# 115dkk/Impulcifer-pip313

Measured on AMD Instinct MI355X. Metric: impulse responses/sec (sweep deconv+FIR), 7.1×2-ear @48kHz, 1/2/4/8 GPU, higher is better.
Workload: dtype f32

## Files before the change

### impulcifer-pip313_amd/csrc/conv_kernels.hip.h

```cpp
#pragma once
#include "fft_regs.hip.h"

namespace imp {

constexpr int kN2 = 4096;
constexpr int kLogN2 = 12;
constexpr int kRowPad = 272;
#ifndef IMP_AB_PREFETCH
#define IMP_AB_PREFETCH 8
#endif
constexpr int kAbPrefetch = IMP_AB_PREFETCH;

struct Twiddles {
  const cf* __restrict__ full;
  const cf* __restrict__ hi;
  const cf* __restrict__ t1;
  const cf* __restrict__ t2;
  const cf* __restrict__ t4;
};

__device__ __forceinline__ void xcd_work_item(int nchan, int& tile, int& chan) {
  const int xcd = blockIdx.x & 7;
  const int slot = blockIdx.x >> 3;
  const int tl = slot / nchan;
// ... 795 lines not shown
#pragma unroll
  for (int q = 1; q < 16; ++q) u[q] = bload_cf(r_t2, vl8, q * 16 * 8);
  fft16<+1>(v);
#pragma unroll
  for (int q = 1; q < 16; ++q) v[q] = cmulc(v[q], u[q]);
  wave_lds_fence();
#pragma unroll
  for (int t2 = 0; t2 < 16; ++t2) buf[hi4 * kRowPad + t2 * 17 + lo4] = v[t2];
  wave_lds_fence();
#pragma unroll
  for (int q = 0; q < 16; ++q) u[q] = buf[hi4 * kRowPad + lo4 * 17 + q];
#pragma unroll
  for (int j2 = 0; j2 < 16; ++j2) v[j2] = bload_cf(r_t4, vo8, j2 * 256 * 8);
  fft16<+1>(u);
#pragma unroll
  for (int j2 = 0; j2 < 16; ++j2) u[j2] = cmulc(u[j2], v[j2]);
  wave_lds_fence();
#pragma unroll
  for (int j2 = 0; j2 < 16; ++j2) buf[hi4 * kRowPad + 16 * j2 + lo4] = u[j2];
  __syncthreads();
#pragma unroll
  for (int a = 0; a < 16; ++a) v[a] = buf[a * kRowPad + t];
  fft16<+1>(v);
#pragma unroll
  for (int j = 0; j < 16; ++j) bstore_cf<IMP_AUX_ROWS_ST>(v[j], r_row, vo8, j * 256 * 8);
}

struct FirBlockArgs {
  const float4* __restrict__ ab;
  long long ab_chan_stride;
  float* __restrict__ out;
  long long out_stride;
  long long out_start, out_len;
  int kp;
  int valid;
  int blocks;
  int first_block;
  int nchan;
};

template <int N1>
struct FirBlockCfg {
  static_assert(N1 == 2 || N1 == 4, "fir_block_kernel holds two or four rows");
  static constexpr int kThreads = 256 * N1;
  static constexpr int kPoints = N1 * kN2;
  static constexpr size_t kLds = sizeof(cf) * N1 * 16 * kRowPad;
  static constexpr int kAbPrefetch = N1 == 4 ? 4 : ::imp::kAbPrefetch;
};
constexpr int kFirBlockPoints = FirBlockCfg<4>::kPoints;
constexpr size_t kFirBlockLds = FirBlockCfg<4>::kLds;

template <class L, class = void> struct LoadHasDeviceLen { static constexpr bool value = false; };
template <class L> struct LoadHasDeviceLen<L, decltype((void)L::kDeviceLen)> { static constexpr bool value = true; };

template <int N1>
__device__ __forceinline__ cf fir_twiddle(__amdgpu_buffer_rsrc_t r_full, int k1, int n2) {
  return bload_cf(r_full, (unsigned)((k1 * (4 / N1)) * kN2 + n2) * 8u, 0u);
}

template <int N1, class Load>
__global__ __launch_bounds__(FirBlockCfg<N1>::kThreads, 4) void fir_block_kernel(Load ld, FirBlockArgs a, Twiddles tw) {
  using Cfg = FirBlockCfg<N1>;
  constexpr int T = Cfg::kThreads;
  extern __shared__ __attribute__((aligned(16))) char smem_raw[];
  cf* lds = reinterpret_cast<cf*>(smem_raw);
  const int xcd = blockIdx.x & 7, slot = blockIdx.x >> 3;
  const int chan = (slot / a.blocks) * 8 + xcd, blk = a.first_block + slot % a.blocks;
  if (chan >= a.nchan) return;
  long long out_len = a.out_len;
  int filt = chan;
  if constexpr (LoadHasDeviceLen<Load>::value) {
    out_len = ld.out_len(chan);
    filt = ld.filter_of(chan);
    if ((long long)blk * a.valid - a.out_start >= out_len) return;
  }
  const int tid = threadIdx.x;
  const int pairq = N1 == 4 ? __builtin_amdgcn_readfirstlane(tid >> 9) : 0;
  const int half = __builtin_amdgcn_readfirstlane((tid >> 8) & 1);
  const int t = tid & 255;
  const int k1 = pairq + (N1 / 2) * half;
  const int s0 = blk * a.valid - a.kp;
  const __amdgpu_buffer_rsrc_t r_full = make_rsrc(tw.full, 4u * kN2 * 8u);
  const auto row = ld.open(chan);

  constexpr int CPT = kN2 / T;
  constexpr int CH = 8 / N1;
  cf v[16];
#pragma unroll
  for (int h = 0; h < CPT / CH; ++h) {
    cf x[CH][N1], w[CH][N1 - 1];
#pragma unroll
    for (int c = 0; c < CH; ++c) {
      const int n2 = tid + T * (CH * h + c);
#pragma unroll
      for (int n1 = 0; n1 < N1; ++n1) x[c][n1] = row.pair_at(s0 + 2 * (n1 * kN2 + n2));
#pragma unroll
      for (int k = 1; k < N1; ++k) w[c][k - 1] = fir_twiddle<N1>(r_full, k, n2);
    }
#pragma unroll
    for (int c = 0; c < CH; ++c) {
      const int n2 = tid + T * (CH * h + c);
#pragma unroll
      for (int n1 = 0; n1 < N1; ++n1) x[c][n1] = row.finish(x[c][n1], s0 + 2 * (n1 * kN2 + n2));
      if constexpr (N1 == 4) bfly4<-1>(x[c][0], x[c][1], x[c][2], x[c][3]);
      else bfly2<-1>(x[c][0], x[c][1]);
      lds[n2] = x[c][0];
#pragma unroll
      for (int k = 1; k < N1; ++k) lds[k * kN2 + n2] = cmul(x[c][k], w[c][k - 1]);
    }
  }
  __syncthreads();
#pragma unroll
  for (int j = 0; j < 16; ++j) v[j] = lds[k1 * kN2 + t + 256 * j];
  __syncthreads();
  const __amdgpu_buffer_rsrc_t r_ab =
      make_rsrc(a.ab + (long long)filt * a.ab_chan_stride + (long long)k1 * kN2, kN2 * sizeof(float4));
  rows_core<0, Cfg::kAbPrefetch>(v, lds + pairq * (2 * 16 * kRowPad), half, pairq, k1, r_ab, tw, t);

  __syncthreads();
#pragma unroll
  for (int j = 0; j < 16; ++j) lds[k1 * kN2 + t + 256 * j] = v[j];
  __syncthreads();
  const __amdgpu_buffer_rsrc_t r_out = make_rsrc(a.out + (long long)chan * a.out_stride, (unsigned)out_len * 4u);
  const int o0 = blk * a.valid - a.kp - (int)a.out_start;
#pragma unroll
  for (int c = 0; c < CPT; ++c) {
    const int n2 = tid + T * c;
    cf y[N1];
#pragma unroll
    for (int k = 0; k < N1; ++k) y[k] = lds[k * kN2 + n2];
#pragma unroll
    for (int k = 1; k < N1; ++k) y[k] = cmulc(y[k], fir_twiddle<N1>(r_full, k, n2));
    if constexpr (N1 == 4) bfly4<+1>(y[0], y[1], y[2], y[3]);
    else bfly2<+1>(y[0], y[1]);
#pragma unroll
    for (int n1 = 0; n1 < N1; ++n1) {
// ... 17 lines not shown
```

### impulcifer-pip313_amd/csrc/impulse_hip.hip

```cpp
#include <hip/hip_runtime.h>

#include <algorithm>
#include <cmath>
#include <complex>
#include <cstdarg>
#include <cstdio>
#include <cstdlib>
#include <cstring>
#include <map>
#include <mutex>
#include <new>
#include <string>
#include <vector>

#include "internal.h"
#include "conv_kernels.hip.h"
#include "ir_kernels.hip.h"
#include "decay_kernels.hip.h"
#include "slice_kernels.hip.h"
#include "vbass_kernels.hip.h"
#include "micdev_kernels.hip.h"

static thread_local std::string g_last_error;

// ... 1674 lines not shown
  return mic_mismatch_impl<float>(ctx, "imp_mic_mismatch_device", d_x, off, len, peak, group, side, anchor, B, G, win, pre, fs, grid,
                                  M, raw_out, power_out);
}

extern "C" int imp_mic_mismatch(imp_ctx* ctx, const double* x, const int64_t* off, const int64_t* len, const int64_t* peak,
                                const int32_t* group, const int32_t* side, const int32_t* anchor, int64_t B, int64_t G, int64_t win,
                                int64_t pre, double fs, const double* grid, int64_t M, double* raw_out, double* power_out) {
  if (!ctx) return fail(IMP_ERR_INVALID, "imp_mic_mismatch: null ctx");
  IMP_CTX_LOCK(ctx);
  int64_t ext = 0;
  int rc = mic_check("imp_mic_mismatch", x, off, len, peak, group, side, anchor, B, G, win, pre, fs, grid, M, raw_out, &ext);
  if (rc || (rc = ctx_bind(ctx))) return rc;
  double* d_x = nullptr;
  if ((rc = ctx_block_get(ctx, (size_t)std::max<int64_t>(ext, 1) * sizeof(double), (void**)&d_x))) return rc;
  if (ext > 0) {
    hipError_t e = hipMemcpyAsync(d_x, x, (size_t)ext * sizeof(double), hipMemcpyHostToDevice, ctx->stream);
    if (e != hipSuccess) {
      (void)hipStreamSynchronize(ctx->stream);
      (void)ctx_block_put(ctx, d_x);
      return fail(IMP_ERR_HIP, "imp_mic_mismatch: h2d: %s", hipGetErrorString(e));
    }
  }
  rc = mic_mismatch_impl<double>(ctx, "imp_mic_mismatch", d_x, off, len, peak, group, side, anchor, B, G, win, pre, fs, grid, M,
                                 raw_out, power_out);
  (void)hipStreamSynchronize(ctx->stream);
  (void)ctx_block_put(ctx, d_x);
  return rc;
}

struct imp_chain {
  imp_ctx* ctx = nullptr;
  imp_ctx* tail_ctx = nullptr;
  imp_plan* deconv = nullptr;
  imp_plan* fir = nullptr;
  int64_t B = 0, n = 0, head = 0, fade_in = 0, fade_out = 0, pitch_ir = 0;
  double peak_height = 0.12589;
  int lanes = 1;
  int sets = 1;
  int64_t calls = 0;
  int tiles = 0;
  int64_t chunks = 0;
  std::vector<float*> d_ir;
  std::vector<unsigned*> d_tile;
  std::vector<imp::RowPeak*> d_res;
  std::vector<hipEvent_t> k1_done;
  std::vector<hipEvent_t> ir_free;
  std::vector<char> ir_busy;
  int64_t* d_meta = nullptr;
  double* d_win = nullptr;
  float4* d_ab2 = nullptr;
  int64_t ab2_gen = -1;
  int t2_kp = 0, t2_valid = 0;
  int64_t t2_first = 0, t2_blocks = 0;
};

static bool chain_tail2_geometry(int64_t M, int64_t out_start, int64_t out_len, int* kp, int* valid, int64_t* first,
                                 int64_t* blocks) {
  if (M < 1 || M > kChainTail2MaxTaps) return false;
  *kp = (int)((M - 1 + 1) & ~(int64_t)1);
  *valid = (int)(2 * imp::FirBlockCfg<2>::kPoints - *kp);
  *first = out_start / *valid;
  *blocks = (out_start + out_len - 1) / *valid - *first + 1;
  return true;
}

static int chain_tail2_prepare(imp_chain* c, bool* ready) {
  imp_plan* f = c->fir;
  *ready = false;
  if (!c->d_ab2) return IMP_OK;
  if (c->ab2_gen == f->filter_gen) {
    *ready = true;
    return IMP_OK;
  }
  if (!f->d_taps || f->taps_gen != f->filter_gen) return IMP_OK;
  int rc = spectrum_alpha_beta_device(f->ctx, f->d_taps, f->M, f->n_filters, f->M, imp::FirBlockCfg<2>::kPoints, 2, c->d_ab2, true);
  if (rc) return rc;
  c->ab2_gen = f->filter_gen;
  *ready = true;
  return IMP_OK;
}

struct ChainLock {
  std::unique_lock<std::recursive_mutex> a, b;
  ChainLock(imp_ctx* x, imp_ctx* y) {
    if (x == y) {
      a = std::unique_lock<std::recursive_mutex>(x->mu);
    } else {
      imp_ctx* lo = x < y ? x : y;
      imp_ctx* hi = x < y ? y : x;
      a = std::unique_lock<std::recursive_mutex>(lo->mu);
      b = std::unique_lock<std::recursive_mutex>(hi->mu);
    }
  }
};

extern "C" void imp_chain_destroy(imp_chain* c) {
  if (!c) return;
  ChainLock lk(c->ctx, c->tail_ctx);
  (void)hipSetDevice(c->ctx->device);
  (void)plan_sync_lanes(c->deconv);
  (void)hipStreamSynchronize(c->tail_ctx->stream);
  for (auto p : c->d_ir) (void)hipFree(p);
  for (auto p : c->d_tile) (void)hipFree(p);
  for (auto p : c->d_res) (void)hipFree(p);
  for (auto e : c->k1_done) (void)hipEventDestroy(e);
  for (auto e : c->ir_free) (void)hipEventDestroy(e);
// ... 30 lines not shown
    return fail(IMP_ERR_UNSUPPORTED, "imp_chain_create: deconvolution plan of %d rows", deconv->N1);
  int rc = ctx_bind(deconv->ctx);
  if (rc) return rc;
  imp_chain* c = new (std::nothrow) imp_chain();
  if (!c) return fail(IMP_ERR_ALLOC, "out of host memory");
  c->ctx = deconv->ctx;
  c->tail_ctx = fir->ctx;
  c->deconv = deconv;
  c->fir = fir;
  c->B = B;
  c->n = n;
  c->head = head;
  c->fade_in = fade_in;
  c->fade_out = fade_out;
  c->peak_height = peak_height;
  c->lanes = deconv->lanes;
  c->sets = deconv->ctx == fir->ctx ? 1 : c->lanes + 1;
  c->pitch_ir = (deconv->out_len + 63) / 64 * 64;
  std::vector<int64_t> meta((size_t)(2 * B));
  for (int64_t b = 0; b < B; ++b) {
    meta[(size_t)b] = b * c->pitch_ir;
    meta[(size_t)(B + b)] = deconv->out_len;
  }
  c->tiles = plan_col_tiles(deconv);
  c->chunks = deconv->paired ? deconv->N1 / 2 : deconv->N1;
  const size_t chunk_bytes = (size_t)(B * c->chunks) * sizeof(unsigned);
  bool ok = hipMalloc((void**)&c->d_meta, (size_t)(2 * B) * sizeof(int64_t)) == hipSuccess &&
            hipMemcpy(c->d_meta, meta.data(), meta.size() * sizeof(int64_t), hipMemcpyHostToDevice) == hipSuccess &&
            hipMalloc((void**)&c->d_win, (size_t)std::max<int64_t>(fade_in + fade_out, 1) * sizeof(double)) == hipSuccess;
  if (ok && fade_in + fade_out > 0) {
    hipLaunchKernelGGL(imp::fade_table_kernel, dim3((unsigned)((fade_in + fade_out + 255) / 256)), dim3(256), 0, deconv->ctx->stream,
                       c->d_win, (long long)fade_in, (long long)fade_out);
    ok = hipGetLastError() == hipSuccess && hipStreamSynchronize(deconv->ctx->stream) == hipSuccess;
  }
  for (int l = 0; l < c->sets && ok; ++l) {
    float* ir = nullptr;
    unsigned* tile = nullptr;
    imp::RowPeak* res = nullptr;
    hipEvent_t e1 = nullptr, e2 = nullptr;
    ok = hipMalloc((void**)&ir, (size_t)(B * c->pitch_ir) * sizeof(float)) == hipSuccess;
    if (ir) c->d_ir.push_back(ir);
    ok = ok && hipMalloc((void**)&tile, chunk_bytes * (size_t)c->tiles) == hipSuccess;
    if (tile) c->d_tile.push_back(tile);
    ok = ok && hipMalloc((void**)&res, (size_t)B * sizeof(imp::RowPeak)) == hipSuccess;
    if (res) c->d_res.push_back(res);
    ok = ok && hipEventCreateWithFlags(&e1, hipEventDisableTiming) == hipSuccess;
    if (e1) c->k1_done.push_back(e1);
    ok = ok && hipEventCreateWithFlags(&e2, hipEventDisableTiming) == hipSuccess;
    if (e2) c->ir_free.push_back(e2);
  }
  c->ir_busy.assign((size_t)c->sets, 0);
  const char* k5_env = std::getenv("IMPULSE_HIP_CHAIN_K5");
  const bool block4 = k5_env && std::strcmp(k5_env, "block4") == 0;
  if (ok && fir->fused && !block4 &&
      chain_tail2_geometry(fir->M, fir->out_start, fir->out_len, &c->t2_kp, &c->t2_valid, &c->t2_first, &c->t2_blocks)) {
    ok = hipMalloc((void**)&c->d_ab2, (size_t)fir->n_filters * imp::FirBlockCfg<2>::kPoints * sizeof(float4)) == hipSuccess;
    bool ready = false;
    if (ok && (rc = chain_tail2_prepare(c, &ready))) {
      imp_chain_destroy(c);
      return rc;
    }
  }
  if (!ok) {
    (void)hipGetLastError();
    imp_chain_destroy(c);
    return fail(IMP_ERR_ALLOC, "imp_chain_create: device allocation failed");
  }
  *out = c;
  return IMP_OK;
}

extern "C" int imp_chain_execute_device(imp_chain* c, const float* d_x, int64_t chan_stride_in, int64_t elem_stride_in,
                                        float* d_out, int64_t chan_stride_out, long long* d_peaks_out) {
  if (!c || !d_x || !d_out) return fail(IMP_ERR_INVALID, "imp_chain_execute_device: null argument");
  ChainLock lk(c->ctx, c->tail_ctx);
  if (chan_stride_out < c->fir->out_len)
    return fail(IMP_ERR_INVALID, "chan_stride_out %lld < out_len %lld", (long long)chan_stride_out, (long long)c->fir->out_len);
  if (c->deconv->lanes != c->lanes || c->fir->lanes != 1)
    return fail(IMP_ERR_INVALID, "imp_chain_execute_device: a plan's overlap setting changed since the chain was made");
  int rc = ctx_bind(c->ctx);
  if (rc) return rc;
  const int lane = c->lanes > 1 ? (int)(c->deconv->group_counter_lane % c->lanes) : 0;
  const int l = (int)(c->calls++ % c->sets);
  hipStream_t lane_stream = lane ? c->ctx->side_streams[(size_t)(lane - 1)] : c->ctx->stream;
  hipStream_t tail = c->tail_ctx->stream;
  if (c->ir_busy[(size_t)l] && tail != lane_stream) HIP_TRY(hipStreamWaitEvent(lane_stream, c->ir_free[(size_t)l], 0));
  c->deconv->tile_max = c->d_tile[(size_t)l];
  rc = imp_conv_execute_device(c->deconv, d_x, c->B, chan_stride_in, elem_stride_in, c->d_ir[(size_t)l], c->pitch_ir);
  c->deconv->tile_max = nullptr;
  if (rc) return rc;
  if (c->deconv->cur_stream != lane_stream) return fail(IMP_ERR_HIP, "imp_chain_execute_device: lane bookkeeping out of step");
  if (tail != lane_stream) {
    HIP_TRY(hipEventRecord(c->k1_done[(size_t)l], lane_stream));
    HIP_TRY(hipStreamWaitEvent(tail, c->k1_done[(size_t)l], 0));
  }
  hipLaunchKernelGGL(imp::row_first_peak_chunked_kernel, dim3((unsigned)c->B), dim3(imp::kPeakThreads), 0, tail, c->d_ir[(size_t)l],
                     c->d_meta, c->d_meta + c->B, c->deconv->out_start, (const unsigned*)c->d_tile[(size_t)l], c->tiles,
                     (const unsigned*)nullptr, c->chunks, c->d_res[(size_t)l], c->peak_height, d_peaks_out);
  HIP_TRY(hipGetLastError());
  imp::LoadCropAtPeak ld{c->d_ir[(size_t)l], c->pitch_ir, c->deconv->out_len, c->d_res[(size_t)l], c->n, c->head, c->fade_in, c->fade_out,
                         c->d_win};
  bool tail2 = false;
  if ((rc = chain_tail2_prepare(c, &tail2))) return rc;
  if (tail2) {
    imp_plan* f = c->fir;
    f->cur_stream = f->ctx->stream;
    if ((rc = timing_event(f, 0))) return rc;
    if ((rc = launch_fir_block_rows<2>(f, ld, c->B, d_out, chan_stride_out, c->d_ab2, c->t2_kp, c->t2_valid, c->t2_first,
                                       c->t2_blocks)))
      return rc;
    for (int slot = 1; slot <= 3; ++slot)
      if ((rc = timing_event(f, slot))) return rc;
  } else if ((rc = run_group_with(c->fir, ld, c->B, d_out, chan_stride_out, 0, 2))) {
    return rc;
  }
  if (tail != lane_stream) {
    HIP_TRY(hipEventRecord(c->ir_free[(size_t)l], tail));
    c->ir_busy[(size_t)l] = 1;
  }
  return IMP_OK;
}

extern "C" int imp_chain_tail_rows(imp_chain* c, int* rows) {
  if (!c || !rows) return fail(IMP_ERR_INVALID, "imp_chain_tail_rows: null argument");
  ChainLock lk(c->ctx, c->tail_ctx);
  imp_plan* f = c->fir;
  *rows = c->d_ab2 && (c->ab2_gen == f->filter_gen || (f->d_taps && f->taps_gen == f->filter_gen)) ? 2 : 4;
  return IMP_OK;
}

extern "C" int imp_debug_chain_tail_geometry(int64_t M, int64_t L, int64_t* history, int64_t* valid, int64_t* blocks) {
  if (L < 1) return fail(IMP_ERR_INVALID, "L must be >= 1 (got %lld)", (long long)L);
  int kp = 0, v = 0;
  int64_t first = 0, nb = 0;
  if (!chain_tail2_geometry(M, 0, L + M - 1, &kp, &v, &first, &nb))
    return fail(IMP_ERR_UNSUPPORTED, "the chain's 2-row K5 takes 1 to %lld taps (got %lld)", (long long)kChainTail2MaxTaps,
                (long long)M);
  if (history) *history = kp;
  if (valid) *valid = v;
  if (blocks) *blocks = nb;
  return IMP_OK;
}

struct imp_segset {
  imp_ctx* ctx = nullptr;
  int64_t B = 0;
  double* e = nullptr;
  int64_t* off = nullptr;
  int64_t* len = nullptr;
  std::vector<int64_t> h_len;
  void* qbuf = nullptr;
  size_t qcap = 0;
  void* keep_a = nullptr;
  void* keep_b = nullptr;
  std::vector<int64_t> keep_host;
};

extern "C" void imp_segset_destroy(imp_segset* s) {
  if (!s) return;
  IMP_CTX_LOCK(s->ctx);
  (void)hipSetDevice(s->ctx->device);
  (void)hipStreamSynchronize(s->ctx->stream);
  (void)ctx_block_put(s->ctx, s->e);
// ... 775 lines not shown
```

### impulcifer-pip313_amd/csrc/ir_kernels.hip.h

```cpp
#pragma once
#include <hip/hip_runtime.h>
#include <stdint.h>

#include "conv_kernels.hip.h"

namespace imp {

struct RowPeak {
  unsigned int maxabs_bits;
  unsigned int pad;
  unsigned long long first_peak;
  unsigned long long first_max;
};

constexpr int kPeakChunk = 8192;
#ifdef IMP_PEAK_DIAG
#define IMP_PEAK_T(k) do { if (threadIdx.x == 0 && blockIdx.x == 0) peak_ts[k] = clock64(); } while (0)
#else
#define IMP_PEAK_T(k) do { } while (0)
#endif
constexpr int kPeakThreads = 1024;
constexpr int kMaxPlanRows = 256;

__device__ __forceinline__ int64_t peak_chunks(int64_t n, int64_t shift) {
// ... 3 lines not shown
template <int NW>
__device__ __forceinline__ float block_max_f32(float m, float* wm ) {
#pragma unroll
  for (int s = 32; s > 0; s >>= 1) m = fmaxf(m, __shfl_xor(m, s, 64));
  __syncthreads();
  if ((threadIdx.x & 63) == 0) wm[threadIdx.x >> 6] = m;
  __syncthreads();
  float r = wm[0];
#pragma unroll
  for (int k = 1; k < NW; ++k) r = fmaxf(r, wm[k]);
  return r;
}

template <int NW>
__device__ __forceinline__ unsigned long long block_min_u64(unsigned long long v, unsigned long long* wm ) {
#pragma unroll
  for (int s = 32; s > 0; s >>= 1) {
    const unsigned long long o = __shfl_xor(v, s, 64);
    v = o < v ? o : v;
  }
  __syncthreads();
  if ((threadIdx.x & 63) == 0) wm[threadIdx.x >> 6] = v;
  __syncthreads();
  unsigned long long r = wm[0];
#pragma unroll
  for (int k = 1; k < NW; ++k) r = wm[k] < r ? wm[k] : r;
  return r;
}

__global__ __launch_bounds__(256) void row_chunk_max_kernel(const float* __restrict__ x, const int64_t* __restrict__ off,
                                                            const int64_t* __restrict__ len, int64_t shift,
                                                            unsigned* __restrict__ chunk_max, int64_t pitch) {
  const int b = blockIdx.y;
  const int64_t n = len[b], c = blockIdx.x;
  if (c >= peak_chunks(n, shift)) return;
  const int64_t lo = c * kPeakChunk - shift > 0 ? c * kPeakChunk - shift : 0;
  const int64_t hi = (c + 1) * kPeakChunk - shift < n ? (c + 1) * kPeakChunk - shift : n;
  const float* row = x + off[b];
  float m = 0.f;
  int64_t i = lo + threadIdx.x;
  for (; i + 7 * 256 < hi; i += 8 * 256) {
    float v[8];
#pragma unroll
    for (int k = 0; k < 8; ++k) v[k] = row[i + k * 256];
#pragma unroll
    for (int k = 0; k < 8; ++k) m = fmaxf(m, fabsf(v[k]));
  }
  for (; i < hi; i += 256) m = fmaxf(m, fabsf(row[i]));
  __shared__ __attribute__((aligned(16))) float wm[4];
  m = block_max_f32<4>(m, wm);
  if (threadIdx.x == 0) chunk_max[(int64_t)b * pitch + c] = __float_as_uint(m);
}

__global__ __launch_bounds__(kPeakThreads) void row_first_peak_chunked_kernel(
    const float* __restrict__ x, const int64_t* __restrict__ off, const int64_t* __restrict__ len, int64_t shift,
    const unsigned* __restrict__ tile_max, int tiles, const unsigned* __restrict__ chunk_max, int64_t pitch,
    RowPeak* __restrict__ res, double height, long long* __restrict__ peaks_out) {
  const int b = blockIdx.x, tid = threadIdx.x;
#ifdef IMP_PEAK_DIAG
  long long peak_ts[8] = {0, 0, 0, 0, 0, 0, 0, 0};
#endif
  IMP_PEAK_T(0);
  const int64_t n = len[b];
  const float* row = x + off[b];
  const int64_t nch = peak_chunks(n, shift);
  constexpr int NW = kPeakThreads / 64;
  __shared__ __attribute__((aligned(16))) float wmf[NW];
  __shared__ __attribute__((aligned(16))) unsigned long long wmu[NW];
  __shared__ float sx[kPeakChunk + 2];
  constexpr int kLdsChunks = 2048;
  __shared__ unsigned srows[kLdsChunks];
  const unsigned* cm = chunk_max + (int64_t)b * pitch;
  if (tiles > 0) {
    for (int r = tid; r < kMaxPlanRows; r += kPeakThreads) srows[r] = 0u;
    __syncthreads();
    const unsigned* tm = tile_max + (int64_t)b * tiles * pitch;
    const int lane = tid & 63, w = tid >> 6;
    for (int64_t r = lane; r < nch; r += 64) {
      unsigned m = 0u;
#pragma unroll 4
      for (int t = w; t < tiles; t += kPeakThreads / 64) {
        const unsigned v = tm[(int64_t)t * pitch + r];
        m = v > m ? v : m;
      }
      if (m) atomicMax(&srows[r], m);
    }
    __syncthreads();
    cm = srows;
  } else if (nch <= kLdsChunks) {
    for (int64_t c = tid; c < nch; c += kPeakThreads) srows[c] = cm[c];
    __syncthreads();
    cm = srows;
  }
  IMP_PEAK_T(1);
  float mf = 0.f;
  for (int64_t c = tid; c < nch; c += kPeakThreads) mf = fmaxf(mf, __uint_as_float(cm[c]));
  const float maxabs = block_max_f32<NW>(mf, wmf);
  RowPeak out;
  out.maxabs_bits = __float_as_uint(maxabs);
  out.pad = 0u;
  out.first_peak = ~0ull;
  out.first_max = ~0ull;
  if (maxabs >= 1e-20f) {
    __shared__ float s_thr;
    if (tid == 0) {
      const double dmax = (double)maxabs;
      float t = (float)(height * dmax);
      if (!(t >= 0.f)) t = 0.f;
      for (int k = 0; k < 4 && t > 0.f && (double)__uint_as_float(__float_as_uint(t) - 1u) / dmax >= height; ++k)
        t = __uint_as_float(__float_as_uint(t) - 1u);
      for (int k = 0; k < 4 && !((double)t / dmax >= height); ++k) t = __uint_as_float(__float_as_uint(t) + 1u);
      s_thr = t;
    }
    __syncthreads();
    const float thr = s_thr;
    IMP_PEAK_T(2);
    unsigned long long c_q = ~0ull;
    for (int64_t c = tid; c < nch; c += kPeakThreads)
      if (__uint_as_float(cm[c]) >= thr && (unsigned long long)c < c_q) c_q = (unsigned long long)c;
    c_q = block_min_u64<NW>(c_q, wmu);
    constexpr int U = (kPeakChunk + kPeakThreads - 1) / kPeakThreads;
    int64_t lo = 0, hi = 0;
    auto stage = [&](int64_t c) {
      lo = c * kPeakChunk - shift > 0 ? c * kPeakChunk - shift : 0;
      hi = (c + 1) * kPeakChunk - shift < n ? (c + 1) * kPeakChunk - shift : n;
      const int64_t cnt = hi - lo + 2;
      float t[U + 1];
#pragma unroll
      for (int u = 0; u <= U; ++u) {
        const int64_t k = tid + (int64_t)u * kPeakThreads, i = lo - 1 + k;
        t[u] = (k < cnt && i >= 0 && i < n) ? row[i] : 0.f;
      }
      __syncthreads();
#pragma unroll
      for (int u = 0; u <= U; ++u) {
        const int64_t k = tid + (int64_t)u * kPeakThreads;
        if (k < cnt) sx[k] = t[u];
      }
      __syncthreads();
    };
    IMP_PEAK_T(3);
    for (int64_t c = c_q == ~0ull ? nch : (int64_t)c_q; c < nch; ++c) {
      if (!(__uint_as_float(cm[c]) >= thr)) continue;
      stage(c);
      IMP_PEAK_T(4);
      float xs[U];
#pragma unroll
      for (int u = 0; u < U; ++u) {
        const int64_t i = lo + tid + (int64_t)u * kPeakThreads;
        xs[u] = i < hi ? sx[i - lo + 1] : 0.f;
      }
      unsigned long long best = ~0ull;
#pragma unroll
      for (int u = 0; u < U; ++u) {
        const int64_t i = lo + tid + (int64_t)u * kPeakThreads;
        const float xi = xs[u];
        if (best != ~0ull || !(fabsf(xi) >= thr) || i >= hi || i == 0 || i >= n - 1) continue;
        const float xm = sx[i - lo];
        const bool up = xm < xi, dn = xm > xi;
        if (!up && !dn) continue;
        if (!((up ? xi : -xi) >= thr)) continue;
        int64_t j = i;
        while (j + 1 < n && (j + 1 <= hi ? sx[j + 1 - lo + 1] : row[j + 1]) == xi) ++j;
        if (j + 1 >= n) continue;
        const float xn = j + 1 <= hi ? sx[j + 1 - lo + 1] : row[j + 1];
        if (up ? (xn < xi) : (xn > xi)) best = (unsigned long long)((i + j) / 2);
      }
      best = block_min_u64<NW>(best, wmu);
      if (best != ~0ull) {
        out.first_peak = best;
        break;
      }
    }
    IMP_PEAK_T(5);
    if (out.first_peak == ~0ull) {
      unsigned long long c_max = ~0ull;
      for (int64_t c = tid; c < nch; c += kPeakThreads)
        if (__uint_as_float(cm[c]) == maxabs && (unsigned long long)c < c_max) c_max = (unsigned long long)c;
      c_max = block_min_u64<NW>(c_max, wmu);
      stage((int64_t)c_max);
      unsigned long long best = ~0ull;
      for (int64_t i = lo + tid; i < hi; i += kPeakThreads)
        if (fabsf(sx[i - lo + 1]) == maxabs) {
          best = (unsigned long long)i;
          break;
        }
      out.first_max = block_min_u64<NW>(best, wmu);
    }
  }
  IMP_PEAK_T(6);
#ifdef IMP_PEAK_DIAG
  if (tid == 0 && b == 0)
    printf("peak phases (clk): entry->fold %lld, max+thr %lld, cq %lld, stage %lld, search %lld, fallback %lld\n", peak_ts[1] - peak_ts[0],
           peak_ts[2] - peak_ts[1], peak_ts[3] - peak_ts[2], peak_ts[4] - peak_ts[3], peak_ts[5] - peak_ts[4], peak_ts[6] - peak_ts[5]);
#endif
  if (tid == 0) {
    res[b] = out;
    if (peaks_out) {
      long long pk;
      if (n == 0 || !(maxabs >= 1e-20f)) pk = 0;
      else pk = (long long)(out.first_peak != ~0ull ? out.first_peak : out.first_max);
      peaks_out[b] = pk;
    }
  }
}

__device__ __forceinline__ double hann_sym_fwd(int64_t i, int64_t N) {
  if (N <= 1) return 1.0;
  return 0.5 - 0.5 * cospi(2.0 * (double)i / (double)(N - 1));
}


__device__ __forceinline__ unsigned* crop_max_lds() {
  __shared__ unsigned rows[kMaxPlanRows];
  return rows;
}

struct StoreRealCropMax {
  StoreRealCrop crop;
  unsigned* __restrict__ tile_max;
  __device__ __forceinline__ __amdgpu_buffer_rsrc_t bind(int b) const { return crop.bind(b); }
  __device__ __forceinline__ void begin(int tid, int threads) const {
    unsigned* rows = crop_max_lds();
    for (int r = tid; r < kMaxPlanRows; r += threads) rows[r] = 0u;
    __syncthreads();
  }
  __device__ __forceinline__ void put(__amdgpu_buffer_rsrc_t r, int b, unsigned e, unsigned step_elems, cf v) const {
    crop.put(r, b, e, step_elems, v);
    const unsigned p = e + step_elems;
    const unsigned i_re = 2u * p - (unsigned)crop.start;
    float m = i_re < (unsigned)crop.len ? fabsf(v.x) : 0.f;
    if (i_re + 1u < (unsigned)crop.len) m = fmaxf(m, fabsf(v.y));
    int mi = __float_as_int(m);
    mi = __float_as_int(fmaxf(__int_as_float(mi), __int_as_float(__builtin_amdgcn_update_dpp(0, mi, 0xB1, 0xF, 0xF, true))));
    mi = __float_as_int(fmaxf(__int_as_float(mi), __int_as_float(__builtin_amdgcn_update_dpp(0, mi, 0x4E, 0xF, 0xF, true))));
    mi = __float_as_int(fmaxf(__int_as_float(mi), __int_as_float(__builtin_amdgcn_update_dpp(0, mi, 0x141, 0xF, 0xF, true))));
    mi = __float_as_int(fmaxf(__int_as_float(mi), __int_as_float(__builtin_amdgcn_update_dpp(0, mi, 0x140, 0xF, 0xF, true))));
    mi = __float_as_int(fmaxf(__int_as_float(mi), __int_as_float(__builtin_amdgcn_update_dpp(0, mi, 0x142, 0xA, 0xF, true))));
    if ((threadIdx.x & 31) == 31 && mi != 0) atomicMax(crop_max_lds() + (p >> 12), (unsigned)mi);
  }
  __device__ __forceinline__ void end(int b, int tile, int tiles, int n1, int tid, int threads) const {
    __syncthreads();
    const unsigned* rows = crop_max_lds();
    unsigned* out = tile_max + ((long long)b * tiles + tile) * n1;
    for (int r = tid; r < n1; r += threads) out[r] = rows[r];
  }
};

__device__ __forceinline__ unsigned* crop_max_lds_r() {
  __shared__ unsigned rows_r[kMaxPlanRows];
  return rows_r;
}

__device__ __forceinline__ int half_wave_max(float m) {
  int mi = __float_as_int(m);
  mi = __float_as_int(fmaxf(__int_as_float(mi), __int_as_float(__builtin_amdgcn_update_dpp(0, mi, 0xB1, 0xF, 0xF, true))));
// ... 1 lines not shown
  mi = __float_as_int(fmaxf(__int_as_float(mi), __int_as_float(__builtin_amdgcn_update_dpp(0, mi, 0x141, 0xF, 0xF, true))));
  mi = __float_as_int(fmaxf(__int_as_float(mi), __int_as_float(__builtin_amdgcn_update_dpp(0, mi, 0x140, 0xF, 0xF, true))));
  mi = __float_as_int(fmaxf(__int_as_float(mi), __int_as_float(__builtin_amdgcn_update_dpp(0, mi, 0x142, 0xA, 0xF, true))));
  return mi;
}

struct StorePairCropMax {
  StorePairCrop crop;
  unsigned* __restrict__ tile_max;
  __device__ __forceinline__ __amdgpu_buffer_rsrc_t bind(int p) const { return crop.bind(p); }
  __device__ __forceinline__ void begin(int tid, int threads) const {
    unsigned *rl = crop_max_lds(), *rr = crop_max_lds_r();
    for (int r = tid; r < kMaxPlanRows; r += threads) rl[r] = rr[r] = 0u;
    __syncthreads();
  }
  __device__ __forceinline__ void put(__amdgpu_buffer_rsrc_t r, int p, unsigned e, unsigned step_elems, cf v) const {
    crop.put(r, p, e, step_elems, v);
    const unsigned n = e + step_elems;
    const bool kept = n - (unsigned)crop.start < (unsigned)crop.len;
    const int ml = half_wave_max(kept ? fabsf(v.x) : 0.f), mr = half_wave_max(kept ? fabsf(v.y) : 0.f);
    if ((threadIdx.x & 31) == 31) {
      if (ml != 0) atomicMax(crop_max_lds() + (n >> 13), (unsigned)ml);
      if (mr != 0) atomicMax(crop_max_lds_r() + (n >> 13), (unsigned)mr);
    }
  }
  __device__ __forceinline__ void end(int p, int tile, int tiles, int n1, int tid, int threads) const {
    __syncthreads();
    const int chunks = n1 >> 1;
    const unsigned *rl = crop_max_lds(), *rr = crop_max_lds_r();
    unsigned* out = tile_max + ((long long)(2 * p) * tiles + tile) * chunks;
    for (int r = tid; r < chunks; r += threads) out[r] = rl[r];
    if (2 * p + 1 < crop.nchan) {
      out += (long long)tiles * chunks;
      for (int r = tid; r < chunks; r += threads) out[r] = rr[r];
    }
  }
};

struct LoadCropAtPeak {
  const float* __restrict__ base;
  long long chan_stride;
  long long row_len;
  const RowPeak* __restrict__ res;
  long long n, head, fade_in, fade_out;
  const double* __restrict__ win;
  __host__ __device__ LoadCropAtPeak shifted(long long, long long) const { return *this; }
  static __device__ __forceinline__ float shaped(float x, long long i, long long n, long long fade_in, long long fade_out,
                                                 const double* __restrict__ win) {
    double g = 1.0;
    if (i < fade_in) g *= win[i];
    if (fade_out > 0 && i >= n - fade_out && i < n) g *= win[fade_in + (i - (n - fade_out))];
    return (float)((double)x * g);
  }
  __device__ __forceinline__ long long crop_start(int b) const {
    const RowPeak rp = res[b];
    long long pk;
    if (row_len == 0 || !(__uint_as_float(rp.maxabs_bits) >= 1e-20f)) pk = 0;
    else pk = (long long)(rp.first_peak != ~0ull ? rp.first_peak : rp.first_max);
    long long start = pk - head;
    if (start > row_len - n) start = row_len - n;
    if (start < 0) start = 0;
    return start;
  }
  struct Row {
    __amdgpu_buffer_rsrc_t r;
    int n, fade_in, fade_out;
    const double* __restrict__ win;
    __device__ __forceinline__ cf pair_at(int s) const { return bload_cf<0>(r, (unsigned)s * 4u, 0u); }
    __device__ __forceinline__ cf finish(cf v, int s) const {
      if ((unsigned)s < (unsigned)n && (s < fade_in || s + 1 >= n - fade_out)) {
        v.x = shaped(v.x, s, n, fade_in, fade_out, win);
        v.y = shaped(v.y, s + 1, n, fade_in, fade_out, win);
      }
      return v;
    }
  };
  __device__ __forceinline__ Row open(int b) const {
    const long long start = crop_start(b), avail = row_len - start;
    return Row{make_rsrc(base + (long long)b * chan_stride + start, (unsigned)(avail < n ? avail : n) * 4u), (int)n, (int)fade_in,
               (int)fade_out, win};
  }
  template <int STEP, int F>
  __device__ __forceinline__ void column(int b, unsigned e0, cf (&v)[F]) const {
    const long long start = crop_start(b), avail = row_len - start;
    const __amdgpu_buffer_rsrc_t r = make_rsrc(base + (long long)b * chan_stride + start, (unsigned)(avail < n ? avail : n) * 4u);
#pragma unroll
    for (int j = 0; j < F; ++j) {
      const u32x2 x = __builtin_amdgcn_raw_buffer_load_b64(r, e0 * 8u, (unsigned)(j * STEP) * 8u, 0);
      v[j] = make_float2(__uint_as_float(x.x), __uint_as_float(x.y));
      const long long i = 2ll * ((long long)e0 + (long long)j * STEP);
      if (i < n && (i < fade_in || i + 1 >= n - fade_out)) {
        v[j].x = shaped(v[j].x, i, n, fade_in, fade_out, win);
        v[j].y = shaped(v[j].y, i + 1, n, fade_in, fade_out, win);
      }
    }
  }
};

__global__ __launch_bounds__(256) void fade_table_kernel(double* __restrict__ win, long long fade_in, long long fade_out) {
  const long long i = (long long)blockIdx.x * blockDim.x + threadIdx.x;
  if (i < fade_in) win[i] = hann_sym_fwd(i, 2 * fade_in);
  else if (i < fade_in + fade_out) win[i] = hann_sym_fwd(fade_out + (i - fade_in), 2 * fade_out);
}

struct WindowParams {
  float gain;
  int64_t fade_in;
  int64_t fade_out;
  int64_t decay_start;
  int64_t decay_half;
  int64_t decay_knee;
  float decay_level_db;
};

__device__ __forceinline__ double hann_sym(int64_t i, int64_t N) {
  if (N <= 1) return 1.0;
  return 0.5 - 0.5 * cospi(2.0 * (double)i / (double)(N - 1));
}

__global__ __launch_bounds__(256) void apply_window_kernel(float* __restrict__ x,
                                                           const int64_t* __restrict__ off,
                                                           const int64_t* __restrict__ len,
                                                           const WindowParams* __restrict__ par) {
  const int b = blockIdx.y;
  const int64_t n = len[b];
  float* row = x + off[b];
  const WindowParams p = par[b];
  for (int64_t i = (int64_t)blockIdx.x * blockDim.x + threadIdx.x; i < n; i += (int64_t)gridDim.x * blockDim.x) {
    double g = (double)p.gain;
    if (i < p.fade_in) g *= hann_sym(i, 2 * p.fade_in);
    if (p.fade_out > 0 && i >= n - p.fade_out)
      g *= hann_sym(p.fade_out + (i - (n - p.fade_out)), 2 * p.fade_out);
    if (p.decay_half >= 0) {
      double w;
      if (i < p.decay_start) w = 1.0;
      else if (i < p.decay_knee) w = hann_sym(p.decay_half + (i - p.decay_start), 2 * p.decay_half);
      else w = 0.0;
      g *= pow(10.0, (w - 1.0) * (-(double)p.decay_level_db) / 20.0);
    }
    row[i] = (float)((double)row[i] * g);
  }
}

__global__ __launch_bounds__(256) void apply_window_copy_kernel(const float* __restrict__ src, const int64_t* __restrict__ src_off,
                                                                float* __restrict__ dst, const int64_t* __restrict__ dst_off,
                                                                const int64_t* __restrict__ len,
                                                                const WindowParams* __restrict__ par) {
  const int b = blockIdx.y;
// ... 537 lines not shown
```

Measured before the change: 361,400.

## Fold row first-peak search into the FIR block kernel prologue

Moves the per-row first-peak search into a device function that every FIR block of a channel runs at its start, using the transform's shared memory. Only the first block writes the peak result, and the crop start is taken from the locally computed peak. This removes the separate peak kernel launch and the dependency between the two kernels on the tail stream. In exchange, the tile-max reduction and peak staging are repeated in every block of a channel. The tile-max fold is also rewritten as a flattened, vectorised load loop, which the standalone kernel uses as well. An environment variable restores the separate launch.

```diff
diff --git a/impulcifer-pip313_amd/csrc/conv_kernels.hip.h b/impulcifer-pip313_amd/csrc/conv_kernels.hip.h
--- a/impulcifer-pip313_amd/csrc/conv_kernels.hip.h
+++ b/impulcifer-pip313_amd/csrc/conv_kernels.hip.h
@@ -871,6 +871,8 @@
 
 template <class L, class = void> struct LoadHasDeviceLen { static constexpr bool value = false; };
 template <class L> struct LoadHasDeviceLen<L, decltype((void)L::kDeviceLen)> { static constexpr bool value = true; };
+template <class L, class = void> struct LoadSearchesPeak { static constexpr bool value = false; };
+template <class L> struct LoadSearchesPeak<L, decltype((void)L::kSearchPeak)> { static constexpr bool value = true; };
 
 template <int N1>
 __device__ __forceinline__ cf fir_twiddle(__amdgpu_buffer_rsrc_t r_full, int k1, int n2) {
@@ -900,7 +902,10 @@
   const int k1 = pairq + (N1 / 2) * half;
   const int s0 = blk * a.valid - a.kp;
   const __amdgpu_buffer_rsrc_t r_full = make_rsrc(tw.full, 4u * kN2 * 8u);
-  const auto row = ld.open(chan);
+  const auto row = [&] {
+    if constexpr (LoadSearchesPeak<Load>::value) return ld.template search_and_open<T>(chan, blk == a.first_block, smem_raw);
+    else return ld.open(chan);
+  }();
 
   constexpr int CPT = kN2 / T;
   constexpr int CH = 8 / N1;
diff --git a/impulcifer-pip313_amd/csrc/impulse_hip.hip b/impulcifer-pip313_amd/csrc/impulse_hip.hip
--- a/impulcifer-pip313_amd/csrc/impulse_hip.hip
+++ b/impulcifer-pip313_amd/csrc/impulse_hip.hip
@@ -1750,6 +1750,7 @@
   int64_t ab2_gen = -1;
   int t2_kp = 0, t2_valid = 0;
   int64_t t2_first = 0, t2_blocks = 0;
+  bool peak_launch = false;
 };
 
 static bool chain_tail2_geometry(int64_t M, int64_t out_start, int64_t out_len, int* kp, int* valid, int64_t* first,
@@ -1886,6 +1887,8 @@
   c->ir_busy.assign((size_t)c->sets, 0);
   const char* k5_env = std::getenv("IMPULSE_HIP_CHAIN_K5");
   const bool block4 = k5_env && std::strcmp(k5_env, "block4") == 0;
+  const char* peak_env = std::getenv("IMPULSE_HIP_CHAIN_PEAK");
+  c->peak_launch = peak_env && std::strcmp(peak_env, "launch") == 0;
   if (ok && fir->fused && !block4 &&
       chain_tail2_geometry(fir->M, fir->out_start, fir->out_len, &c->t2_kp, &c->t2_valid, &c->t2_first, &c->t2_blocks)) {
     ok = hipMalloc((void**)&c->d_ab2, (size_t)fir->n_filters * imp::FirBlockCfg<2>::kPoints * sizeof(float4)) == hipSuccess;
@@ -1928,21 +1931,29 @@
     HIP_TRY(hipEventRecord(c->k1_done[(size_t)l], lane_stream));
     HIP_TRY(hipStreamWaitEvent(tail, c->k1_done[(size_t)l], 0));
   }
-  hipLaunchKernelGGL(imp::row_first_peak_chunked_kernel, dim3((unsigned)c->B), dim3(imp::kPeakThreads), 0, tail, c->d_ir[(size_t)l],
-                     c->d_meta, c->d_meta + c->B, c->deconv->out_start, (const unsigned*)c->d_tile[(size_t)l], c->tiles,
-                     (const unsigned*)nullptr, c->chunks, c->d_res[(size_t)l], c->peak_height, d_peaks_out);
-  HIP_TRY(hipGetLastError());
+  bool tail2 = false;
+  if ((rc = chain_tail2_prepare(c, &tail2))) return rc;
+  const bool fold = tail2 && !c->peak_launch;
+  if (!fold) {
+    hipLaunchKernelGGL(imp::row_first_peak_chunked_kernel, dim3((unsigned)c->B), dim3(imp::kPeakThreads), 0, tail, c->d_ir[(size_t)l],
+                       c->d_meta, c->d_meta + c->B, c->deconv->out_start, (const unsigned*)c->d_tile[(size_t)l], c->tiles,
+                       (const unsigned*)nullptr, c->chunks, c->d_res[(size_t)l], c->peak_height, d_peaks_out);
+    HIP_TRY(hipGetLastError());
+  }
   imp::LoadCropAtPeak ld{c->d_ir[(size_t)l], c->pitch_ir, c->deconv->out_len, c->d_res[(size_t)l], c->n, c->head, c->fade_in, c->fade_out,
                          c->d_win};
-  bool tail2 = false;
-  if ((rc = chain_tail2_prepare(c, &tail2))) return rc;
   if (tail2) {
     imp_plan* f = c->fir;
     f->cur_stream = f->ctx->stream;
     if ((rc = timing_event(f, 0))) return rc;
-    if ((rc = launch_fir_block_rows<2>(f, ld, c->B, d_out, chan_stride_out, c->d_ab2, c->t2_kp, c->t2_valid, c->t2_first,
-                                       c->t2_blocks)))
-      return rc;
+    if (fold) {
+      const imp::LoadCropAtPeakSearch lds{ld, c->d_res[(size_t)l], d_peaks_out, c->d_tile[(size_t)l], c->tiles, c->chunks,
+                                          c->deconv->out_start, c->peak_height};
+      rc = launch_fir_block_rows<2>(f, lds, c->B, d_out, chan_stride_out, c->d_ab2, c->t2_kp, c->t2_valid, c->t2_first, c->t2_blocks);
+    } else {
+      rc = launch_fir_block_rows<2>(f, ld, c->B, d_out, chan_stride_out, c->d_ab2, c->t2_kp, c->t2_valid, c->t2_first, c->t2_blocks);
+    }
+    if (rc) return rc;
     for (int slot = 1; slot <= 3; ++slot)
       if ((rc = timing_event(f, slot))) return rc;
   } else if ((rc = run_group_with(c->fir, ld, c->B, d_out, chan_stride_out, 0, 2))) {
diff --git a/impulcifer-pip313_amd/csrc/ir_kernels.hip.h b/impulcifer-pip313_amd/csrc/ir_kernels.hip.h
--- a/impulcifer-pip313_amd/csrc/ir_kernels.hip.h
+++ b/impulcifer-pip313_amd/csrc/ir_kernels.hip.h
@@ -79,49 +79,59 @@
   if (threadIdx.x == 0) chunk_max[(int64_t)b * pitch + c] = __float_as_uint(m);
 }
 
-__global__ __launch_bounds__(kPeakThreads) void row_first_peak_chunked_kernel(
-    const float* __restrict__ x, const int64_t* __restrict__ off, const int64_t* __restrict__ len, int64_t shift,
-    const unsigned* __restrict__ tile_max, int tiles, const unsigned* __restrict__ chunk_max, int64_t pitch,
-    RowPeak* __restrict__ res, double height, long long* __restrict__ peaks_out) {
-  const int b = blockIdx.x, tid = threadIdx.x;
+constexpr int kLdsChunks = 2048;
+constexpr size_t kPeakLdsWmu = 0;
+constexpr size_t kPeakLdsWmf = kPeakLdsWmu + 16 * sizeof(unsigned long long);
+constexpr size_t kPeakLdsThr = kPeakLdsWmf + 16 * sizeof(float);
+constexpr size_t kPeakLdsRows = kPeakLdsThr + 16;
+constexpr size_t kPeakLdsX = kPeakLdsRows + kLdsChunks * sizeof(unsigned);
+constexpr size_t kPeakLdsBytes = kPeakLdsX + (kPeakChunk + 2) * sizeof(float);
+
+template <int T>
+__device__ __forceinline__ RowPeak row_first_peak(const float* __restrict__ row, int64_t n, int64_t shift,
+                                                  const unsigned* __restrict__ tile_max, int tiles,
+                                                  const unsigned* __restrict__ chunk_max, int64_t pitch, double height,
+                                                  char* __restrict__ lds ) {
+  static_assert(T % 64 == 0 && T / 64 <= 16, "row_first_peak: one to sixteen waves");
+  const int tid = threadIdx.x;
 #ifdef IMP_PEAK_DIAG
   long long peak_ts[8] = {0, 0, 0, 0, 0, 0, 0, 0};
 #endif
   IMP_PEAK_T(0);
-  const int64_t n = len[b];
-  const float* row = x + off[b];
   const int64_t nch = peak_chunks(n, shift);
-  constexpr int NW = kPeakThreads / 64;
-  __shared__ __attribute__((aligned(16))) float wmf[NW];
-  __shared__ __attribute__((aligned(16))) unsigned long long wmu[NW];
-  __shared__ float sx[kPeakChunk + 2];
-  constexpr int kLdsChunks = 2048;
-  __shared__ unsigned srows[kLdsChunks];
-  const unsigned* cm = chunk_max + (int64_t)b * pitch;
+  constexpr int NW = T / 64;
+  unsigned long long* wmu = reinterpret_cast<unsigned long long*>(lds + kPeakLdsWmu);
+  float* wmf = reinterpret_cast<float*>(lds + kPeakLdsWmf);
+  float* s_thr = reinterpret_cast<float*>(lds + kPeakLdsThr);
+  unsigned* srows = reinterpret_cast<unsigned*>(lds + kPeakLdsRows);
+  float* sx = reinterpret_cast<float*>(lds + kPeakLdsX);
+  const unsigned* cm = chunk_max;
   if (tiles > 0) {
-    for (int r = tid; r < kMaxPlanRows; r += kPeakThreads) srows[r] = 0u;
-    __syncthreads();
-    const unsigned* tm = tile_max + (int64_t)b * tiles * pitch;
-    const int lane = tid & 63, w = tid >> 6;
-    for (int64_t r = lane; r < nch; r += 64) {
-      unsigned m = 0u;
-#pragma unroll 4
-      for (int t = w; t < tiles; t += kPeakThreads / 64) {
-        const unsigned v = tm[(int64_t)t * pitch + r];
-        m = v > m ? v : m;
-      }
-      if (m) atomicMax(&srows[r], m);
+    for (int r = tid; r < kMaxPlanRows; r += T) srows[r] = 0u;
+    __syncthreads();
+    constexpr int V = 8192 / T;
+    const int rows = (int)nch, words = tiles * rows;
+    for (int f0 = tid; f0 < words; f0 += V * T) {
+      unsigned v[V];
+#pragma unroll
+      for (int q = 0; q < V; ++q) {
+        const int f = f0 + q * T;
+        v[q] = f < words ? tile_max[(int64_t)(f / rows) * pitch + f % rows] : 0u;
+      }
+#pragma unroll
+      for (int q = 0; q < V; ++q)
+        if (v[q]) atomicMax(&srows[(f0 + q * T) % rows], v[q]);
     }
     __syncthreads();
     cm = srows;
   } else if (nch <= kLdsChunks) {
-    for (int64_t c = tid; c < nch; c += kPeakThreads) srows[c] = cm[c];
+    for (int64_t c = tid; c < nch; c += T) srows[c] = cm[c];
     __syncthreads();
     cm = srows;
   }
   IMP_PEAK_T(1);
   float mf = 0.f;
-  for (int64_t c = tid; c < nch; c += kPeakThreads) mf = fmaxf(mf, __uint_as_float(cm[c]));
+  for (int64_t c = tid; c < nch; c += T) mf = fmaxf(mf, __uint_as_float(cm[c]));
   const float maxabs = block_max_f32<NW>(mf, wmf);
   RowPeak out;
   out.maxabs_bits = __float_as_uint(maxabs);
@@ -129,7 +139,6 @@
   out.first_peak = ~0ull;
   out.first_max = ~0ull;
   if (maxabs >= 1e-20f) {
-    __shared__ float s_thr;
     if (tid == 0) {
       const double dmax = (double)maxabs;
       float t = (float)(height * dmax);
@@ -137,31 +146,34 @@
       for (int k = 0; k < 4 && t > 0.f && (double)__uint_as_float(__float_as_uint(t) - 1u) / dmax >= height; ++k)
         t = __uint_as_float(__float_as_uint(t) - 1u);
       for (int k = 0; k < 4 && !((double)t / dmax >= height); ++k) t = __uint_as_float(__float_as_uint(t) + 1u);
-      s_thr = t;
-    }
-    __syncthreads();
-    const float thr = s_thr;
+      *s_thr = t;
+    }
+    __syncthreads();
+    const float thr = *s_thr;
     IMP_PEAK_T(2);
     unsigned long long c_q = ~0ull;
-    for (int64_t c = tid; c < nch; c += kPeakThreads)
+    for (int64_t c = tid; c < nch; c += T)
       if (__uint_as_float(cm[c]) >= thr && (unsigned long long)c < c_q) c_q = (unsigned long long)c;
     c_q = block_min_u64<NW>(c_q, wmu);
-    constexpr int U = (kPeakChunk + kPeakThreads - 1) / kPeakThreads;
+    constexpr int U = (kPeakChunk + T - 1) / T;
     int64_t lo = 0, hi = 0;
     auto stage = [&](int64_t c) {
       lo = c * kPeakChunk - shift > 0 ? c * kPeakChunk - shift : 0;
       hi = (c + 1) * kPeakChunk - shift < n ? (c + 1) * kPeakChunk - shift : n;
-      const int64_t cnt = hi - lo + 2;
+      const int cnt = (int)(hi - lo) + 2;
+      const int k_lo = lo == 0 ? 1 : 0;
+      const int k_hi = n - lo + 1 < cnt ? (int)(n - lo + 1) : cnt;
+      const float* src = row + lo;
       float t[U + 1];
 #pragma unroll
       for (int u = 0; u <= U; ++u) {
-        const int64_t k = tid + (int64_t)u * kPeakThreads, i = lo - 1 + k;
-        t[u] = (k < cnt && i >= 0 && i < n) ? row[i] : 0.f;
+        const int k = tid + u * T;
+        t[u] = (k >= k_lo && k < k_hi) ? src[k - 1] : 0.f;
       }
       __syncthreads();
 #pragma unroll
       for (int u = 0; u <= U; ++u) {
-        const int64_t k = tid + (int64_t)u * kPeakThreads;
+        const int k = tid + u * T;
         if (k < cnt) sx[k] = t[u];
       }
       __syncthreads();
@@ -171,18 +183,22 @@
       if (!(__uint_as_float(cm[c]) >= thr)) continue;
       stage(c);
       IMP_PEAK_T(4);
+      const int span = (int)(hi - lo);
+      const int k_end = n - 1 - lo < span ? (int)(n - 1 - lo) : span;
+      const int k_first = lo == 0 ? 1 : 0;
       float xs[U];
 #pragma unroll
       for (int u = 0; u < U; ++u) {
-        const int64_t i = lo + tid + (int64_t)u * kPeakThreads;
-        xs[u] = i < hi ? sx[i - lo + 1] : 0.f;
+        const int k = tid + u * T;
+        xs[u] = k < span ? sx[k + 1] : 0.f;
       }
       unsigned long long best = ~0ull;
 #pragma unroll
       for (int u = 0; u < U; ++u) {
-        const int64_t i = lo + tid + (int64_t)u * kPeakThreads;
+        const int k = tid + u * T;
         const float xi = xs[u];
-        if (best != ~0ull || !(fabsf(xi) >= thr) || i >= hi || i == 0 || i >= n - 1) continue;
+        if (best != ~0ull || !(fabsf(xi) >= thr) || k < k_first || k >= k_end) continue;
+        const int64_t i = lo + k;
         const float xm = sx[i - lo];
         const bool up = xm < xi, dn = xm > xi;
         if (!up && !dn) continue;
@@ -202,12 +218,12 @@
     IMP_PEAK_T(5);
     if (out.first_peak == ~0ull) {
       unsigned long long c_max = ~0ull;
-      for (int64_t c = tid; c < nch; c += kPeakThreads)
+      for (int64_t c = tid; c < nch; c += T)
         if (__uint_as_float(cm[c]) == maxabs && (unsigned long long)c < c_max) c_max = (unsigned long long)c;
       c_max = block_min_u64<NW>(c_max, wmu);
       stage((int64_t)c_max);
       unsigned long long best = ~0ull;
-      for (int64_t i = lo + tid; i < hi; i += kPeakThreads)
+      for (int64_t i = lo + tid; i < hi; i += T)
         if (fabsf(sx[i - lo + 1]) == maxabs) {
           best = (unsigned long long)i;
           break;
@@ -217,18 +233,30 @@
   }
   IMP_PEAK_T(6);
 #ifdef IMP_PEAK_DIAG
-  if (tid == 0 && b == 0)
+  if (tid == 0 && blockIdx.x == 0)
     printf("peak phases (clk): entry->fold %lld, max+thr %lld, cq %lld, stage %lld, search %lld, fallback %lld\n", peak_ts[1] - peak_ts[0],
            peak_ts[2] - peak_ts[1], peak_ts[3] - peak_ts[2], peak_ts[4] - peak_ts[3], peak_ts[5] - peak_ts[4], peak_ts[6] - peak_ts[5]);
 #endif
-  if (tid == 0) {
+  return out;
+}
+
+__device__ __forceinline__ long long row_peak_index(const RowPeak& rp, int64_t n) {
+  if (n == 0 || !(__uint_as_float(rp.maxabs_bits) >= 1e-20f)) return 0;
+  return (long long)(rp.first_peak != ~0ull ? rp.first_peak : rp.first_max);
+}
+
+__global__ __launch_bounds__(kPeakThreads) void row_first_peak_chunked_kernel(
+    const float* __restrict__ x, const int64_t* __restrict__ off, const int64_t* __restrict__ len, int64_t shift,
+    const unsigned* __restrict__ tile_max, int tiles, const unsigned* __restrict__ chunk_max, int64_t pitch,
+    RowPeak* __restrict__ res, double height, long long* __restrict__ peaks_out) {
+  __shared__ __attribute__((aligned(16))) char lds[kPeakLdsBytes];
+  const int b = blockIdx.x;
+  const int64_t n = len[b];
+  const RowPeak out = row_first_peak<kPeakThreads>(x + off[b], n, shift, tile_max + (int64_t)b * tiles * pitch, tiles,
+                                                   chunk_max + (int64_t)b * pitch, pitch, height, lds);
+  if (threadIdx.x == 0) {
     res[b] = out;
-    if (peaks_out) {
-      long long pk;
-      if (n == 0 || !(maxabs >= 1e-20f)) pk = 0;
-      else pk = (long long)(out.first_peak != ~0ull ? out.first_peak : out.first_max);
-      peaks_out[b] = pk;
-    }
+    if (peaks_out) peaks_out[b] = row_peak_index(out, n);
   }
 }
 
@@ -336,16 +364,13 @@
     if (fade_out > 0 && i >= n - fade_out && i < n) g *= win[fade_in + (i - (n - fade_out))];
     return (float)((double)x * g);
   }
-  __device__ __forceinline__ long long crop_start(int b) const {
-    const RowPeak rp = res[b];
-    long long pk;
-    if (row_len == 0 || !(__uint_as_float(rp.maxabs_bits) >= 1e-20f)) pk = 0;
-    else pk = (long long)(rp.first_peak != ~0ull ? rp.first_peak : rp.first_max);
+  __device__ __forceinline__ long long start_at(long long pk) const {
     long long start = pk - head;
     if (start > row_len - n) start = row_len - n;
     if (start < 0) start = 0;
     return start;
   }
+  __device__ __forceinline__ long long crop_start(int b) const { return start_at(row_peak_index(res[b], row_len)); }
   struct Row {
     __amdgpu_buffer_rsrc_t r;
     int n, fade_in, fade_out;
@@ -359,11 +384,12 @@
       return v;
     }
   };
-  __device__ __forceinline__ Row open(int b) const {
-    const long long start = crop_start(b), avail = row_len - start;
+  __device__ __forceinline__ Row open_at(int b, long long start) const {
+    const long long avail = row_len - start;
     return Row{make_rsrc(base + (long long)b * chan_stride + start, (unsigned)(avail < n ? avail : n) * 4u), (int)n, (int)fade_in,
                (int)fade_out, win};
   }
+  __device__ __forceinline__ Row open(int b) const { return open_at(b, crop_start(b)); }
   template <int STEP, int F>
   __device__ __forceinline__ void column(int b, unsigned e0, cf (&v)[F]) const {
     const long long start = crop_start(b), avail = row_len - start;
@@ -378,6 +404,36 @@
         v[j].y = shaped(v[j].y, i + 1, n, fade_in, fade_out, win);
       }
     }
+  }
+};
+
+struct LoadCropAtPeakSearch {
+  static constexpr bool kSearchPeak = true;
+  LoadCropAtPeak crop;
+  RowPeak* __restrict__ res;
+  long long* __restrict__ peaks_out;
+  const unsigned* __restrict__ tile_max;
+  int tiles;
+  long long pitch;
+  long long shift;
+  double height;
+  using Row = LoadCropAtPeak::Row;
+  __host__ __device__ LoadCropAtPeakSearch shifted(long long, long long) const { return *this; }
+  template <int T>
+  __device__ __forceinline__ Row search_and_open(int b, bool writer, char* lds) const {
+    static_assert(kPeakLdsBytes <= FirBlockCfg<T / 256>::kLds, "the search needs more LDS than the transform has");
+    const RowPeak rp = row_first_peak<T>(crop.base + (long long)b * crop.chan_stride, crop.row_len, shift,
+                                         tile_max + (long long)b * tiles * pitch, tiles, nullptr, pitch, height, lds);
+    const long long pk = row_peak_index(rp, crop.row_len);
+    if (writer && threadIdx.x == 0) {
+      res[b] = rp;
+      if (peaks_out) peaks_out[b] = pk;
+    }
+    __syncthreads();
+    const long long s = crop.start_at(pk);
+    const long long start = (long long)(((unsigned long long)(unsigned)__builtin_amdgcn_readfirstlane((int)(s >> 32)) << 32) |
+                                        (unsigned)__builtin_amdgcn_readfirstlane((int)s));
+    return crop.open_at(b, start);
   }
 };
 
```

After: 350,400, median of 2. 0.97x the previous value.
